# anshulahuja98/antidote

Measured on AMD Instinct MI355X. Metric: materialized ops/sec + VC compares/sec (1/2/4/8 GPU), % of HBM roofline, higher is better.
Workload: dtype u64; 1 GPU; cfg2 counter_pn materialize: 10M keys x 64 ops/key, 8-DC clocks, random snapshot VCs; keys_per_gpu=10000000, keys_total=10000000, ops_per_key=64, n_dcs=8, r_jitter=U[-2000,2000], partitioning=vnode p = key mod 64, gpu = p mod G; no collective, parallelism=dp1

## Files before the change

### antidote_amd/_abi.py

```python
from __future__ import annotations

import ctypes as C

ABI_VERSION = 7

OK = 0
EINVAL, EHIP, ENOMEM, ECAPACITY, ENOTSUP, ERCCL, ENODEV = -1, -2, -3, -4, -5, -6, -7

COUNTER_PN, SET_AW, REGISTER_MV = 1, 2, 3
TYPE_MIXED = 0xFF
EFFECT_INVALID = -(1 << 63)
TAG_INVALID = 0xFFFFFFFF

F_NEWSS, F_CT_IGNORE, F_ERR_UNEXPECTED, F_ERR_CORRUPTED, F_ERR_CAPACITY = 0x1, 0x2, 0x4, 0x8, 0x10
F_CT_FULL = 0x20
HINT_R_FULL, HINT_CT_FLAG, HINT_MIXED = 0x1, 0x2, 0x4
OPS_THRESHOLD = 50
RESIZE_THRESHOLD = 5
GC_ALL_PRUNED = 0x1
UNIQUE_ID_BYTES = 128
U64_MAX = (1 << 64) - 1

TYPE_NAMES = {
    COUNTER_PN: "antidote_crdt_counter_pn",
# ... 105 lines not shown
    "agn_dev_alloc": (C.c_int, [P, C.c_size_t, C.POINTER(P)]),
    "agn_dev_free": (C.c_int, [P, P]),
    "agn_memcpy_h2d": (C.c_int, [P, P, P, C.c_size_t, P]),
    "agn_memcpy_d2h": (C.c_int, [P, P, P, C.c_size_t, P]),
    "agn_memset_d": (C.c_int, [P, P, C.c_int, C.c_size_t, P]),
    "agn_stream_sync": (C.c_int, [P, P]),
    "agn_materialize": (C.c_int, [P, C.POINTER(AgnLog), C.POINTER(AgnRead),
                                  C.POINTER(AgnResult), P]),
    "agn_materialize_host": (C.c_int, [P, C.POINTER(AgnLog), C.POINTER(AgnRead),
                                       C.POINTER(AgnResult)]),
    "agn_state_capacity": (C.c_int, [C.POINTER(AgnLog), C.POINTER(AgnRead), P]),
    "agn_log_index_ids": (C.c_int, [P, C.POINTER(AgnLog), P, P]),
    "agn_log_index_masks": (C.c_int, [P, C.POINTER(AgnLog), P, P]),
    "agn_log_index_pack": (C.c_int, [P, C.POINTER(AgnLog), P, P, P, C.POINTER(C.c_uint64), P]),
    "agn_log_index_pack16": (C.c_int, [P, C.POINTER(AgnLog), P, P, C.POINTER(C.c_uint64), P]),
    "agn_tune": (C.c_int, [P, C.POINTER(AgnLog), C.POINTER(AgnRead), C.POINTER(AgnResult), P,
                           C.c_int, C.POINTER(C.c_int), P]),
    "agn_select_base": (C.c_int, [P, C.c_uint32, C.c_uint64, P, P, P, P, P, P, P, P]),
    "agn_gst_min": (C.c_int, [P, C.c_uint32, C.c_uint64, C.c_uint64, P, P, P, P]),
    "agn_gst_finalize": (C.c_int, [P, C.c_uint32, C.c_uint64, P, P]),
    "agn_update_stable": (C.c_int, [C.c_uint32, P, P, C.POINTER(C.c_int)]),
    "agn_log_ingest": (C.c_int, [P, C.POINTER(AgnLogRecords), C.c_uint32, C.c_uint32,
                                 C.c_uint64, P, P, C.c_uint32, C.POINTER(AgnLog), P, P]),
    "agn_ss_lookup": (C.c_int, [P, C.POINTER(AgnSsCache), C.c_uint64, P, P, P, P, P, P, P, P,
                                P, P]),
    "agn_ss_store": (C.c_int, [P, C.POINTER(AgnSsCache), C.POINTER(AgnLog), C.c_uint64, P, P, P,
                               P, C.POINTER(AgnResult), P, P, P, P, P]),
    "agn_ss_state_compact": (C.c_int, [P, C.POINTER(AgnSsCache), P, P, C.c_uint64, P]),
    "agn_read_cached": (C.c_int, [P, C.POINTER(AgnSsCache), C.POINTER(AgnLog), C.c_uint64, P, P,
                                  P, P, C.POINTER(AgnResult), P, P, P, P]),
# ... 47 lines not shown
    "oracle_select_base": (C.c_int, [C.c_uint32, C.c_uint64, P, P, P, P, P, P, P]),
    "oracle_log_ingest": (C.c_int, [C.POINTER(AgnLogRecords), C.c_uint32, C.c_uint32,
                                    C.c_uint64, P, P, C.c_uint32, C.POINTER(AgnLog)]),
    "oracle_ss_lookup": (C.c_int, [C.POINTER(AgnSsCache), C.c_uint64, P, P, P, P, P, P, P, P,
                                   P]),
    "oracle_ss_store": (C.c_int, [C.POINTER(AgnSsCache), C.POINTER(AgnLog), C.c_uint64, P, P,
                                  P, P, C.POINTER(AgnResult), P, P, P, P]),
    "oracle_prune_ops": (C.c_int, [C.POINTER(AgnLog), P, P, P, C.POINTER(AgnLog), P]),
    "oracle_gst_scalar": (C.c_int, [C.c_uint32, C.c_uint64, P, P]),
    "oracle_dep_check": (C.c_int, [C.c_uint32, C.c_uint64, P, P, P, P, C.c_uint64, P, P, P]),
    "oracle_vc_le": (C.c_int, [C.c_uint32, P, P, P, P]),
    "oracle_vc_all_dots_greater": (C.c_int, [C.c_uint32, P, P, P, P]),
}


ADDITIVE = frozenset({"agn_log_index_pack16"})


def bind(lib, protos):
    for name, (res, args) in protos.items():
        if name in ADDITIVE and not hasattr(lib, name):
            continue
        fn = getattr(lib, name)
        fn.restype = res
        fn.argtypes = args
    return lib
```

### antidote_amd/csrc/api.hip

```cpp
#include <hip/hip_runtime.h>
#include <hipcub/hipcub.hpp>
#include <rccl/rccl.h>

#include <algorithm>
#include <atomic>
#include <cstdarg>
#include <cstdio>
#include <cstdlib>
#include <cstring>
#include <mutex>
#include <string>
#include <thread>
#include <vector>

#include "common.hpp"
#include "gen.hpp"
#include "serve.hpp"

namespace agn {
struct Stager {
    hipStream_t s = nullptr;
    char *d = nullptr, *h = nullptr;
    size_t cap = 0;
};
// ... 125 lines not shown
    std::lock_guard<std::mutex> g(ctx->mi_mu);
    for (const auto &m : ctx->mi)
        if (m.key_mask == log->key_mask && m.n_keys == log->n_keys)
            return many_mixed(m.mixed, m.n_keys);
    return false;
}

namespace {
struct PackEnt {
    agn_ctx *ctx;
    const uint64_t *oc, *key_off;
    uint64_t n_entries, n_keys, seq;
    PackIdx idx;
    bool owned;
    bool owned16;
};
constexpr int kPackIdx = 16;
std::mutex g_pk_mu;
PackEnt g_pk[kPackIdx] = {};
uint64_t g_pk_seq = 0;
std::atomic<int> g_pk_live{0};

void pack_drop16_locked(PackEnt &e) {
    if (e.owned16) {
        (void)hipFree((void *)e.idx.rows16);
        (void)hipFree((void *)e.idx.narrow);
    }
    e.idx.rows16 = nullptr;
    e.idx.narrow = nullptr;
    e.idx.n_wide = 0;
    e.owned16 = false;
}

void pack_drop_locked(PackEnt &e) {
    if (!e.ctx) return;
    pack_drop16_locked(e);
    if (e.owned) {
        (void)hipFree((void *)e.idx.rows);
// ... 17 lines not shown
}

void pack_register(agn_ctx *ctx, const agn_log &log, const PackIdx &idx, bool owned) {
    std::lock_guard<std::mutex> g(g_pk_mu);
    PackEnt *slot = nullptr;
    for (auto &e : g_pk)
        if (pack_match(e, log)) slot = &e;
    for (auto &e : g_pk)
        if (!slot && !e.ctx) slot = &e;
    if (!slot) {
        slot = &g_pk[0];
        for (auto &e : g_pk)
            if (e.seq < slot->seq) slot = &e;
    }
    pack_drop_locked(*slot);
    *slot = {ctx, log.oc, log.key_off, log.n_entries, log.n_keys, ++g_pk_seq, idx, owned, false};
    g_pk_live.fetch_add(1, std::memory_order_release);
}

void pack_unregister16(const agn_log &log) {
    if (g_pk_live.load(std::memory_order_relaxed) == 0) return;
    std::lock_guard<std::mutex> g(g_pk_mu);
    for (auto &e : g_pk)
        if (pack_match(e, log)) pack_drop16_locked(e);
}

bool pack_register16(const agn_log &log, const uint16_t *rows16, const uint8_t *narrow,
                     uint64_t n_wide, bool owned) {
    std::lock_guard<std::mutex> g(g_pk_mu);
    for (auto &e : g_pk)
        if (pack_match(e, log)) {
            pack_drop16_locked(e);
            e.idx.rows16 = rows16;
            e.idx.narrow = narrow;
            e.idx.n_wide = n_wide;
            e.owned16 = owned;
            return true;
        }
    return false;
}

void pack_clear(agn_ctx *ctx) {
    if (g_pk_live.load(std::memory_order_relaxed) == 0) return;
    std::lock_guard<std::mutex> g(g_pk_mu);
    for (auto &e : g_pk)
        if (e.ctx == ctx) pack_drop_locked(e);
}

void pack_forget(const void *p) {
    if (g_pk_live.load(std::memory_order_relaxed) == 0) return;
    std::lock_guard<std::mutex> g(g_pk_mu);
    for (auto &e : g_pk) {
        if (!e.ctx) continue;
        if (p == e.oc || p == e.key_off || p == e.idx.rows || p == e.idx.base || p == e.idx.ok)
            pack_drop_locked(e);
        else if (e.idx.rows16 && (p == e.idx.rows16 || p == e.idx.narrow))
            pack_drop16_locked(e);
    }
}
}

bool pack_lookup(const agn_log &log, PackIdx *out) {
    if (g_pk_live.load(std::memory_order_relaxed) == 0) return false;
    std::lock_guard<std::mutex> g(g_pk_mu);
    for (const auto &e : g_pk)
        if (pack_match(e, log)) {
            *out = e.idx;
            return true;
        }
    return false;
}

// ... 277 lines not shown
    if (log->crdt_type != AGN_COUNTER_PN || log->n_dcs != 8 || log->oc_mask)
        return fail(AGN_ENOTSUP, "index_pack16: counter_pn logs with 8 dense DCs only");
    if (!narrow) return fail(AGN_EINVAL, "index_pack16: narrow required");
    if (((uintptr_t)rows16 & 15u) || misaligned4(narrow))
        return fail(AGN_EINVAL, "index_pack16: rows16 16-byte, narrow 4-byte aligned");
    PackIdx pk{};
    if (!pack_lookup(*log, &pk))
        return fail(AGN_EINVAL, "index_pack16: no packed index registered for the log "
                                "(agn_log_index_pack first)");
    uint64_t wide = 0;
    rc = launch_index_pack16(*log, pk.rows, pk.ok, rows16, narrow, &wide, (hipStream_t)stream);
    if (rc) return rc;
    if (n_wide) *n_wide = wide;
    if (!pack_register16(*log, rows16, narrow, wide, false))
        return fail(AGN_EINVAL, "index_pack16: the log's packed index was dropped meanwhile");
    return AGN_OK;
}

int agn_state_capacity(const agn_log *log, const agn_read *req, uint64_t *cap_off) {
    if (!log || !req || !cap_off) return fail(AGN_EINVAL, "null argument");
    cap_off[0] = 0;
    for (uint64_t i = 0; i < req->n_req; ++i) {
        const uint64_t k = req->keys ? req->keys[i] : i;
        uint64_t c = 0;
        if (log->add_tok)
            for (uint64_t e = log->key_off[k]; e < log->key_off[k] + key_n(log->key_off, log->key_len, k); ++e)
                c += log->add_tok[e] != 0;
        if (req->base_off) c += req->base_off[i + 1] - req->base_off[i];
        else if (req->base_value && is_tag_type(log->crdt_type))
            c += AGN_SS_STATE_PAIRS(req->base_value[i]);
// ... 779 lines not shown
            pack_register(ctx, *log, PackIdx{(uint32_t *)pr, (uint64_t *)pb, (uint8_t *)po}, true);
            void *p16 = nullptr, *pn = nullptr;
            uint64_t wide = 0;
            const bool tier =
                hipMalloc(&p16, E * 8 * sizeof(uint16_t)) == hipSuccess &&
                hipMalloc(&pn, (K + 7) / 8 * 8) == hipSuccess &&
                launch_index_pack16(*log, (const uint32_t *)pr, (const uint8_t *)po, (uint16_t *)p16,
                                    (uint8_t *)pn, &wide, s) == AGN_OK &&
                pack_register16(*log, (const uint16_t *)p16, (const uint8_t *)pn, wide, true);
            if (!tier) {
                (void)hipGetLastError();
                (void)hipStreamSynchronize(s);
                if (p16) (void)hipFree(p16);
                if (pn) (void)hipFree(pn);
            }
        } else {
            (void)hipGetLastError();
            (void)hipStreamSynchronize(s);
            if (pr) (void)hipFree(pr);
            if (pb) (void)hipFree(pb);
            if (po) (void)hipFree(po);
        }
    }
    (void)hipStreamSynchronize(s);
    (void)hipFree(scratch);
    if (he != hipSuccess) err = fail(AGN_EHIP, "k_gen: %s", hipGetErrorString(he));
    if (err) agn_gen_free_dev(ctx, log, req);
    return err;
}

// ... 126 lines not shown
```

### antidote_amd/csrc/common.hpp

```cpp
#pragma once

#include <hip/hip_runtime.h>
#include <stdint.h>
#include <stdlib.h>

#include <atomic>
#include <shared_mutex>

#include "../../include/antidote_gpu.h"

#define AGN_WAVE 64

namespace agn {

extern std::atomic<uint32_t> g_env_gen;
class EnvKnob {
  public:
    explicit EnvKnob(const char *name) : name_(name) {}
    const char *get() {
        const uint32_t g = g_env_gen.load(std::memory_order_acquire);
        if (gen_.load(std::memory_order_acquire) != g) refresh(g);
        return val_.load(std::memory_order_acquire);
    }

// ... 189 lines not shown
                     uint64_t *mixed = nullptr);
void oplog_view(const agn_oplog *L, agn_log *v);
agn_ctx *oplog_ctx(const agn_oplog *L);

int launch_counter(const agn_log &log, const agn_read &req, const agn_result &out,
                   hipStream_t s);
int launch_index_ids(const agn_log &log, uint32_t *out, hipStream_t st);
int launch_index_masks(const agn_log &log, uint64_t *out, uint64_t *mixed, hipStream_t st);
struct PackIdx {
    const uint32_t *rows;
    const uint64_t *base;
    const uint8_t *ok;
    const uint16_t *rows16;
    const uint8_t *narrow;
    uint64_t n_wide;
};
int launch_index_pack(const agn_log &log, uint32_t *rows, uint64_t *base, uint8_t *ok,
                      uint64_t *n_unpacked, hipStream_t st);
int launch_index_pack16(const agn_log &log, const uint32_t *rows, const uint8_t *ok,
                        uint16_t *rows16, uint8_t *narrow, uint64_t *n_wide, hipStream_t st);
bool pack_lookup(const agn_log &log, PackIdx *out);
int launch_counter_dense(const agn_log &log, const agn_read &req, const agn_result &out,
                         hipStream_t s);
int tune_counter_dense(const agn_log &log, const agn_read &req, const agn_result &out,
                       hipStream_t st, int rounds, int *choice, float *ms);
int launch_tags(const agn_log &log, const agn_read &req, const agn_result &out,
                hipStream_t s);
int launch_gst_min(uint32_t D, uint64_t P, uint64_t E, const uint64_t *clocks,
                   const uint8_t *defined, uint64_t *out, hipStream_t s);
int launch_gst_finalize(uint32_t D, uint64_t E, uint64_t *vec, hipStream_t s);
int launch_log_ingest(const agn_log_records &r, uint32_t D, uint64_t n_keys,
                      const uint64_t *max_t, const uint64_t *max_m, uint32_t base,
                      const agn_log &out, uint64_t *totals, hipStream_t st);
int launch_ss_lookup(const agn_ss_cache &c, uint64_t n_req, const uint64_t *keys,
                     const uint64_t *R, const uint64_t *Rm, uint64_t *sct, uint64_t *sctm,
// ... 35 lines not shown
```

### antidote_amd/csrc/counter_scan.hpp

```cpp
#pragma once
#include "common.hpp"

namespace agn {
namespace {

__device__ __forceinline__ uint64_t dpp_u64(uint64_t v, int ctrl_id) {
    uint32_t lo = (uint32_t)v, hi = (uint32_t)(v >> 32);
    switch (ctrl_id) {
        case 0:
            lo = __builtin_amdgcn_update_dpp(0u, lo, 0xB1, 0xF, 0xF, false);
            hi = __builtin_amdgcn_update_dpp(0u, hi, 0xB1, 0xF, 0xF, false);
            break;
        case 1:
            lo = __builtin_amdgcn_update_dpp(0u, lo, 0x4E, 0xF, 0xF, false);
            hi = __builtin_amdgcn_update_dpp(0u, hi, 0x4E, 0xF, 0xF, false);
            break;
        case 2:
            lo = __builtin_amdgcn_update_dpp(0u, lo, 0x141, 0xF, 0xF, false);
            hi = __builtin_amdgcn_update_dpp(0u, hi, 0x141, 0xF, 0xF, false);
            break;
        default:
            lo = __builtin_amdgcn_update_dpp(0u, lo, 0x140, 0xF, 0xF, false);
            hi = __builtin_amdgcn_update_dpp(0u, hi, 0x140, 0xF, 0xF, false);
            break;
// ... 513 lines not shown
        return keep + shfl_xor_u64(send, stride);
    };
    const bool b5 = (lane & 32) != 0, b4 = (lane & 16) != 0, b3 = (lane & 8) != 0;
    uint64_t v4[4], v2[2];
#pragma unroll
    for (int k = 0; k < 4; ++k) v4[k] = xch(b5 ? s[4 + k] : s[k], b5 ? s[k] : s[4 + k], 32);
#pragma unroll
    for (int k = 0; k < 2; ++k) v2[k] = xch(b4 ? v4[2 + k] : v4[k], b4 ? v4[k] : v4[2 + k], 16);
    uint64_t v = xch(b3 ? v2[1] : v2[0], b3 ? v2[0] : v2[1], 8);
    v += dpp_u64(v, 0);
    v += dpp_u64(v, 1);
    v += dpp_u64(v, 2);
    return v;
}

typedef unsigned long long u64x4 __attribute__((ext_vector_type(4)));
typedef u64x4 u64x4_a8 __attribute__((aligned(8)));
typedef u32x4 u32x4_a4 __attribute__((aligned(4)));
__device__ __forceinline__ u64x4 ldc_u64x4(const uint64_t *p) {
    return *(const __attribute__((address_space(4))) u64x4_a8 *)p;
}
__device__ __forceinline__ u32x4 ldc_u32x4(const uint32_t *p) {
    return *(const __attribute__((address_space(4))) u32x4_a4 *)p;
}

template <bool WARM, bool NT, bool EFF_NT = false, bool FROM1 = false>
__device__ __forceinline__ void scan_key_q8(
    const uint64_t *__restrict__ oc, const int64_t *__restrict__ eff,
    const uint64_t *__restrict__ txid, uint64_t txr, uint64_t off, uint64_t n,
    uint64_t n_entries, uint64_t rA, uint64_t rB, uint64_t sA, uint64_t sB, uint64_t &ctA,
// ... 64 lines not shown
```

### antidote_amd/csrc/mat_counter_dense.hip

```cpp
#include <atomic>
#include <cstdlib>
#include <vector>

#include "counter_scan.hpp"

namespace agn {
namespace {

constexpr uint32_t QL_S = 1024, QL_STRIDE = 32;

inline uint32_t counter_order(uint64_t n_req, uint32_t bulk) {
    return order_or(n_req < (1ull << 20) ? 1u : bulk);
}
constexpr uint32_t BULK_CHUNK = 64;
constexpr uint32_t BULK_CHUNK4 = 64;
constexpr bool Q2_FOUR_DEFAULT = true;
constexpr uint32_t BULK_CHUNK8 = 64;
constexpr uint64_t NARROW_WIDE_DIV = 1024;

struct DenseArgs {
    uint64_t n_req;
    uint64_t n_entries;
    uint32_t req_type;
    uint32_t xcd;
    uint32_t pair;
    uint32_t qnt;
    uint32_t hints;
    uint32_t ql_cap;
};

struct MaskArgs {
    const uint64_t *key_mask, *oc_mask, *R_mask, *sct_mask;
    uint64_t *o_mask;
// ... 1117 lines not shown
    const uint64_t left = a.n_req - i0;
    const uint32_t m = left < 4u ? (uint32_t)left : 4u;
#pragma nounroll
    for (uint32_t h = 0; h < m; ++h) q2_serve_oc(a, i0 + h);
}

struct Q2Pack8Params {
    DenseArgs a;
    MaskArgs mk;
    const void *args[20];
    const uint32_t *rows;
    const uint64_t *base;
    const uint8_t *ok;
    const uint16_t *rows16;
    const uint8_t *narrow;
};
static_assert(offsetof(Q2Pack8Params, rows) == offsetof(Q2PackParams, rows) &&
                  offsetof(Q2Pack8Params, base) == offsetof(Q2PackParams, base),
              "Q2Pack8Params extends Q2PackParams");

__global__ __launch_bounds__(64) void k_counter_pack8(Q2Pack8Params) {
    const DenseArgs a = dense_of(kparams<Q2Params>().a);
    const uint32_t blk = block_order(a.xcd, blockIdx.x, gridDim.x);
    const uint64_t i0 = uniform_u64((uint64_t)blk * 8u);
    if (i0 >= a.n_req) return;
    const int lane = lane_id();
    if (i0 + 7u < a.n_req) {
        const auto &pm = kparams<Q2Params>();
        const uint64_t *const key_off = pm.key_off, *const key_len = pm.key_len;
        const uint32_t *const key_id0 = pm.key_id0;
        const uint8_t *const key_type = pm.key_type;
        const uint64_t *const R = pm.R;
        const int64_t *const bvp = pm.base_value;
        const auto &pq = *(const __attribute__((address_space(4))) Q2Pack8Params *)&pm;
        const uint64_t *const pbase = pq.base;
// ... 19 lines not shown
        const uint64_t v_n64 = has_len ? v_lr : v_nx - v_off;
        const uint32_t v_n = (uint32_t)v_n64;
        const uint32_t v_id0 = has_id0 ? v_ir : AGN_ID0_NONE;
        const uint32_t kt = (((lane & 4) ? ktw1 : ktw0) >> (8u * ((uint32_t)lane & 3u))) & 0xffu;
        const uint32_t want = key_type != nullptr ? (a.req_type & 0xffu) : kt;
        const bool lbad = lane < 8 && (v_n64 > (uint64_t)AGN_WAVE || (v_n64 != 0 && kt != want));
        const bool bad = ballot(lbad) != 0ull || nw0 != 0x01010101u || nw1 != 0x01010101u ||
                         a.n_entries == 0;
        if (!bad) {
            const uint16_t *const rows16 = kparams<Q2Pack8Params>().rows16;
            u32x4 c[8];
#pragma unroll
            for (int g = 0; g < 8; ++g)
                c[g] = n8_load_rows<true>(rows16, n8_readlane_u64(v_off, g), a.n_entries);
            const int64_t *const l_eff = kparams<Q2Params>().eff;
            __builtin_amdgcn_sched_barrier(0);
            const uint64_t below = ballot(rv < bv);
            const uint64_t dl = rv - bv;
            const uint32_t tp = n8_thr_pack(dl > 0xFFFFull ? 0xFFFFu : (uint32_t)dl);
            uint32_t v_cnt = 0, v_fx = 0, v_fe = 0, v_inc = 0;
            uint32_t cg = 0;
            const int kg = lane >> 3;
            int64_t ev[8];
#pragma unroll
            for (int g = 0; g < 8; ++g) {
                const uint32_t th0 = __builtin_amdgcn_readlane(tp, 8 * g);
                const uint32_t th1 = __builtin_amdgcn_readlane(tp, 8 * g + 2);
                const uint32_t th2 = __builtin_amdgcn_readlane(tp, 8 * g + 4);
                const uint32_t th3 = __builtin_amdgcn_readlane(tp, 8 * g + 6);
                const uint32_t noR = (uint32_t)(below >> (8 * g)) & 0xFFu;
                const uint32_t n_g = __builtin_amdgcn_readlane(v_n, g);
                const uint64_t off_g = n8_readlane_u64(v_off, g);
                const bool valid = (uint32_t)lane < n_g;
                const bool ex = (noR | n8_excl(c[g], th0, th1, th2, th3)) != 0u;
                const bool mine = valid & !ex;
                const uint64_t exm = ballot(valid & ex);
                const uint32_t cnt = (uint32_t)__builtin_popcountll(ballot(mine));
                const uint32_t fx = exm ? (uint32_t)__builtin_ctzll(exm) : 0xFFFFFFFFu;
                ev[g] = n8_load_eff(l_eff, off_g, mine,
                                    reinterpret_cast<const int64_t *>(R + (i0 + (uint64_t)g) * 8u));
                c[g].x = mine ? c[g].x : 0u;
                c[g].y = mine ? c[g].y : 0u;
                c[g].z = mine ? c[g].z : 0u;
                c[g].w = mine ? c[g].w : 0u;
                v_inc |= mine ? (1u << g) : 0u;
                __builtin_amdgcn_sched_barrier(0);
                cg = kg == g ? cnt : cg;
                v_cnt = put_lane(cnt, g, v_cnt);
                v_fx = put_lane(fx, g, v_fx);
            }
            __builtin_amdgcn_sched_barrier(0);
            const auto &pr = kparams<Q2Params>();
            const uint32_t *const l_op_id = pr.op_id;
            int64_t *const l_value = pr.o_value, *const l_hole = pr.o_hole;
            uint64_t *const l_lastct = pr.o_lastct;
            uint32_t *const l_count = pr.o_count, *const l_flags = pr.o_flags, *const l_err = pr.o_err;
            const int32_t fx = (int32_t)v_fx;
            const uint32_t pos = fx >= 0 ? (uint32_t)fx : v_n - 1u;
            const bool need = lane < 8 && v_id0 == AGN_ID0_NONE && v_n != 0u;
            const uint32_t *const ip = need ? l_op_id + (v_off + (uint64_t)pos)
                                            : reinterpret_cast<const uint32_t *>(R + slot);
            const uint32_t opid = *ip;
            const uint32_t md = n8_maxfold(c);
            const uint64_t ct = cg ? bv + (uint64_t)md : 0ull;
            __builtin_amdgcn_sched_barrier(0);
            uint64_t sm[8];
#pragma unroll
            for (int g = 0; g < 8; ++g) {
                const bool mine = ((v_inc >> g) & 1u) != 0u;
                const bool badv = mine && ev[g] == AGN_EFFECT_INVALID;
                const uint64_t be = ballot(badv);
                v_fe = put_lane(be ? (uint32_t)__builtin_ctzll(be) : 0xFFFFFFFFu, g, v_fe);
                sm[g] = (mine && !badv) ? (uint64_t)ev[g] : 0ull;
            }
            const uint64_t ks = n8_sumfold(sm);
            const uint64_t total =
                ((uint64_t)(uint32_t)__shfl((int)(uint32_t)(ks >> 32), 8 * (int)m8, AGN_WAVE) << 32) |
                (uint32_t)__shfl((int)(uint32_t)ks, 8 * (int)m8, AGN_WAVE);
            __builtin_amdgcn_sched_barrier(0);
            const uint64_t idh = v_id0 != AGN_ID0_NONE ? (uint64_t)v_id0 + (uint64_t)pos : (uint64_t)opid;
            const int64_t hid = v_n ? (int64_t)idh : 0;
            const int32_t fe = (int32_t)v_fe;
            uint32_t fl = v_cnt ? AGN_F_NEWSS : AGN_F_CT_IGNORE;
            fl |= fe >= 0 ? AGN_F_ERR_UNEXPECTED : 0u;
            l_lastct[slot] = ct;
            if (lane < 8) {
                const uint64_t i = i0 + (uint64_t)lane;
                l_value[i] = (int64_t)(reqbase + total);
                l_hole[i] = fx >= 0 ? hid - 1 : hid;
                l_count[i] = v_cnt;
                l_err[i] = fe >= 0 ? (uint32_t)(v_off + (uint64_t)fe) : 0xffffffffu;
                l_flags[i] = fl;
            }
// ... 204 lines not shown
                          (uintptr_t)mk.o_mask;
    const uintptr_t a8 = (uintptr_t)out.count | (uintptr_t)out.flags | (uintptr_t)out.err_pos;
    const bool q2s = ((sv && (sv[0] == '0' || sv[0] == '1')) ? sv[0] == '1' : dflt) &&
                     (a16 & 15u) == 0 && (a8 & 7u) == 0;
    const char *pv = AGN_KNOB("AGN_Q2_PACK");
    const bool pack = dflt && q2e && q2s && log.n_entries != 0 && !(pv && pv[0] == '0') &&
                      pack_lookup(log, &pk);
    const char *fv = AGN_KNOB("AGN_Q2_FOUR");
    const bool four = pack && !req.keys && log.n_entries / 64u <= log.n_keys &&
                      ((fv && (fv[0] == '0' || fv[0] == '1')) ? fv[0] == '1' : Q2_FOUR_DEFAULT);
    const char *nv = AGN_KNOB("AGN_Q2_NARROW");
    const bool eight = four && pk.rows16 && pk.narrow &&
                       ((nv && (nv[0] == '0' || nv[0] == '1'))
                            ? nv[0] == '1'
                            : pk.n_wide * NARROW_WIDE_DIV <= log.n_keys);
    if (eight) {
        a.xcd = counter_order(req.n_req, BULK_CHUNK8);
        const Q2Pack8Params p{a, mk,
                              {req.keys, log.key_off, log.key_len, log.key_type, id0_index(log),
                               log.oc, log.op_id, log.eff, log.txid, req.R, req.sct, req.sct_ignore,
                               req.txid, req.base_value, out.value, out.hole, out.lastct, out.count,
                               out.flags, out.err_pos},
                              pk.rows, pk.base, pk.ok, pk.rows16, pk.narrow};
        hipLaunchKernelGGL(k_counter_pack8, dim3((unsigned)((req.n_req + 7) / 8)), dim3(64), 0, st, p);
    } else if (four) {
        a.xcd = counter_order(req.n_req, BULK_CHUNK4);
        const Q2PackParams p{a, mk,
                             {req.keys, log.key_off, log.key_len, log.key_type, id0_index(log),
                              log.oc, log.op_id, log.eff, log.txid, req.R, req.sct, req.sct_ignore,
                              req.txid, req.base_value, out.value, out.hole, out.lastct, out.count,
                              out.flags, out.err_pos},
                             pk.rows, pk.base, pk.ok};
        hipLaunchKernelGGL(k_counter_pack4, dim3((unsigned)((req.n_req + 3) / 4)), dim3(64), 0, st, p);
    } else if (pack) {
        AGN_Q2L_(false, false, true, true, true);
    } else if (req.sct) {
        if (msk) AGN_Q2L(true, true);
        else AGN_Q2L(true, false);
    } else {
// ... 352 lines not shown
                    u32x4 v;
                    v.x = lo.x | (lo.y << 16);
                    v.y = lo.z | (lo.w << 16);
                    v.z = hh.x | (hh.y << 16);
                    v.w = hh.z | (hh.w << 16);
                    reinterpret_cast<u32x4 *>(rows16)[off + p] = v;
                }
            }
        }
    }
    __syncthreads();
    if (threadIdx.x == 0 && blk_w)
        atomicAdd(&wide[(blockIdx.x % IM_CNT) * IM_STRIDE], (unsigned long long)blk_w);
}

}

int launch_index_pack16(const agn_log &log, const uint32_t *rows, const uint8_t *ok,
                        uint16_t *rows16, uint8_t *narrow, uint64_t *n_wide, hipStream_t st) {
    const uint64_t nb = (log.n_keys + 3) / 4;
    *n_wide = 0;
    if (nb == 0) return AGN_OK;
    if (nb > 0x7fffffffull) return fail(AGN_EINVAL, "index_pack16: too many keys");
    unsigned long long *cnt = nullptr;
    const size_t cb = (size_t)IM_CNT * IM_STRIDE * sizeof(unsigned long long);
    AGN_HIP(pool_malloc(&cnt, cb, st));
    if (hipMemsetAsync(cnt, 0, cb, st) != hipSuccess) {
        (void)hipFreeAsync(cnt, st);
        return fail(AGN_EHIP, "index_pack16: counter reset");
    }
// ... 165 lines not shown
```

### antidote_amd/engine.py

```python
from __future__ import annotations

import ctypes as C
from dataclasses import dataclass, field

import numpy as np

from . import _abi
from ._lib import EngineUnavailable, check, load
from .encode import (EncodedLog, EncodedRead, ResultArrays, alloc_result, log_struct, n_words,
                     read_struct, result_struct)


class DevBuf:

    def __init__(self, eng: "Engine", nbytes: int):
        self.eng, self.nbytes = eng, int(nbytes)
        p = C.c_void_p()
        check(eng.lib.agn_dev_alloc(eng.ctx, self.nbytes, C.byref(p)), "agn_dev_alloc")
        self.ptr = p.value or 0
        eng._bufs.add(self)

    def free(self):
        if self.ptr:
            self.eng.lib.agn_dev_free(self.eng.ctx, self.ptr)
# ... 115 lines not shown
        ls = dlog.struct if isinstance(dlog, DeviceArrays) else dlog
        K, E = int(ls.n_keys), int(ls.n_entries)
        rows16, narrow = self.empty(max(1, E) * 16), self.empty(max(1, (K + 7) // 8) * 8)
        n = C.c_uint64(0)
        check(self.lib.agn_log_index_pack16(self.ctx, C.byref(ls), rows16.ptr, narrow.ptr,
                                            C.byref(n), stream),
              "agn_log_index_pack16")
        if isinstance(dlog, DeviceArrays):
            dlog.bufs.update(pack_rows16=rows16, pack_narrow=narrow)
        return rows16, narrow, n.value

    def drop_pack16(self, dlog):
        ls = dlog.struct if isinstance(dlog, DeviceArrays) else dlog
        check(self.lib.agn_log_index_pack16(self.ctx, C.byref(ls), None, None, None, None),
              "agn_log_index_pack16")

    def drop_pack(self, dlog):
        ls = dlog.struct if isinstance(dlog, DeviceArrays) else dlog
        check(self.lib.agn_log_index_pack(self.ctx, C.byref(ls), None, None, None, None, None),
              "agn_log_index_pack")

    def alloc_log_like(self, log: EncodedLog) -> DeviceArrays:
        s = _abi.AgnLog()
        s.crdt_type, s.n_dcs = log.crdt_type, log.n_dcs
        s.n_keys, s.n_entries = log.n_keys, log.n_entries
        d = DeviceArrays(s)
        for name in ("key_off", "oc", "oc_mask", "op_id", "txid", "eff", "tag", "add_tok",
                     "rem_off", "rem_tok"):
            a = getattr(log, name)
            if a is None or (isinstance(a, np.ndarray) and a.size == 0 and name != "rem_tok"):
# ... 395 lines not shown
```

### include/antidote_gpu.h

```cpp
#ifndef ANTIDOTE_GPU_H
#define ANTIDOTE_GPU_H

#include <stddef.h>
#include <stdint.h>

#ifdef __cplusplus
extern "C" {
#endif

#define AGN_ABI_VERSION 7

#define AGN_OK 0
#define AGN_EINVAL (-1)
#define AGN_EHIP (-2)
#define AGN_ENOMEM (-3)
#define AGN_ECAPACITY (-4)
#define AGN_ENOTSUP (-5)
#define AGN_ERCCL (-6)
#define AGN_ENODEV (-7)

#define AGN_COUNTER_PN 1
#define AGN_SET_AW 2
#define AGN_REGISTER_MV 3
#define AGN_TYPE_MIXED 0xFF
// ... 92 lines not shown
int agn_materialize_host(agn_ctx *ctx, const agn_log *log, const agn_read *req,
                         agn_result *out);

int agn_tune(agn_ctx *ctx, const agn_log *log, const agn_read *req, agn_result *out,
             void *stream, int rounds, int *choice, float *ms);

int agn_log_index_ids(agn_ctx *ctx, const agn_log *log, uint32_t *out, void *stream);

int agn_log_index_masks(agn_ctx *ctx, const agn_log *log, uint64_t *out, void *stream);

int agn_log_index_pack(agn_ctx *ctx, const agn_log *log, uint32_t *rows, uint64_t *base,
                       uint8_t *ok, uint64_t *n_unpacked, void *stream);

int agn_log_index_pack16(agn_ctx *ctx, const agn_log *log, uint16_t *rows16, uint8_t *narrow,
                         uint64_t *n_wide, void *stream);

int agn_state_capacity(const agn_log *host_log, const agn_read *host_req,
                       uint64_t *cap_off);

#define AGN_OPS_THRESHOLD 50
#define AGN_RESIZE_THRESHOLD 5
typedef struct agn_oplog agn_oplog;
int agn_oplog_create(agn_ctx *ctx, uint32_t crdt_type, uint32_t n_dcs, uint64_t n_keys,
                     int sparse, uint32_t init_slots, agn_oplog **out);
int agn_oplog_destroy(agn_oplog *log);
int agn_oplog_append(agn_oplog *log, uint64_t n, const uint64_t *keys, const uint8_t *same_op,
                     const uint64_t *oc, const uint64_t *oc_mask, const uint64_t *txid,
                     const int64_t *eff, const uint32_t *tag, const uint64_t *add_tok,
                     const uint32_t *rem_off, const uint64_t *rem_tok, uint32_t *out_op_id,
                     uint8_t *out_gc_due);
// ... 187 lines not shown
```

Before: 228.9 billion ops/s.

## Add cached int16 effect tier with escape fallback for 8-DC counter materialize

Adds a derived int16 copy of the counter effect column. Values outside ±32767 are marked with a sentinel and counted. The eight-DC packed materialize kernel gets a templated path that loads the 2-byte effects and sums them in 32 bits with a new shuffle/DPP fold. It falls back to the 64-bit effect array only for escaped entries, which also keeps the invalid-effect error check there. The goal is to cut HBM traffic for effects; the cost is an extra index build, a host sync to count escapes, and more registry bookkeeping.

```diff
diff --git a/antidote_amd/_abi.py b/antidote_amd/_abi.py
--- a/antidote_amd/_abi.py
+++ b/antidote_amd/_abi.py
@@ -143,6 +143,7 @@
     "agn_log_index_masks": (C.c_int, [P, C.POINTER(AgnLog), P, P]),
     "agn_log_index_pack": (C.c_int, [P, C.POINTER(AgnLog), P, P, P, C.POINTER(C.c_uint64), P]),
     "agn_log_index_pack16": (C.c_int, [P, C.POINTER(AgnLog), P, P, C.POINTER(C.c_uint64), P]),
+    "agn_log_index_eff16": (C.c_int, [P, C.POINTER(AgnLog), P, C.POINTER(C.c_uint64), P]),
     "agn_tune": (C.c_int, [P, C.POINTER(AgnLog), C.POINTER(AgnRead), C.POINTER(AgnResult), P,
                            C.c_int, C.POINTER(C.c_int), P]),
     "agn_select_base": (C.c_int, [P, C.c_uint32, C.c_uint64, P, P, P, P, P, P, P, P]),
@@ -220,7 +221,7 @@
 }
 
 
-ADDITIVE = frozenset({"agn_log_index_pack16"})
+ADDITIVE = frozenset({"agn_log_index_pack16", "agn_log_index_eff16"})
 
 
 def bind(lib, protos):
diff --git a/antidote_amd/csrc/api.hip b/antidote_amd/csrc/api.hip
--- a/antidote_amd/csrc/api.hip
+++ b/antidote_amd/csrc/api.hip
@@ -163,6 +163,7 @@
     PackIdx idx;
     bool owned;
     bool owned16;
+    bool owned_e;
 };
 constexpr int kPackIdx = 16;
 std::mutex g_pk_mu;
@@ -170,7 +171,16 @@
 uint64_t g_pk_seq = 0;
 std::atomic<int> g_pk_live{0};
 
+void pack_drop_eff_locked(PackEnt &e) {
+    if (e.owned_e) (void)hipFree((void *)e.idx.eff16);
+    e.idx.eff16 = nullptr;
+    e.idx.eff_src = nullptr;
+    e.idx.n_esc = 0;
+    e.owned_e = false;
+}
+
 void pack_drop16_locked(PackEnt &e) {
+    pack_drop_eff_locked(e);
     if (e.owned16) {
         (void)hipFree((void *)e.idx.rows16);
         (void)hipFree((void *)e.idx.narrow);
@@ -218,7 +228,7 @@
             if (e.seq < slot->seq) slot = &e;
     }
     pack_drop_locked(*slot);
-    *slot = {ctx, log.oc, log.key_off, log.n_entries, log.n_keys, ++g_pk_seq, idx, owned, false};
+    *slot = {ctx, log.oc, log.key_off, log.n_entries, log.n_keys, ++g_pk_seq, idx, owned, false, false};
     g_pk_live.fetch_add(1, std::memory_order_release);
 }
 
@@ -244,6 +254,27 @@
     return false;
 }
 
+void pack_unregister_eff(const agn_log &log) {
+    if (g_pk_live.load(std::memory_order_relaxed) == 0) return;
+    std::lock_guard<std::mutex> g(g_pk_mu);
+    for (auto &e : g_pk)
+        if (pack_match(e, log)) pack_drop_eff_locked(e);
+}
+
+bool pack_register_eff(const agn_log &log, const int16_t *eff16, uint64_t n_esc, bool owned) {
+    std::lock_guard<std::mutex> g(g_pk_mu);
+    for (auto &e : g_pk)
+        if (pack_match(e, log) && e.idx.rows16) {
+            pack_drop_eff_locked(e);
+            e.idx.eff16 = eff16;
+            e.idx.eff_src = log.eff;
+            e.idx.n_esc = n_esc;
+            e.owned_e = owned;
+            return true;
+        }
+    return false;
+}
+
 void pack_clear(agn_ctx *ctx) {
     if (g_pk_live.load(std::memory_order_relaxed) == 0) return;
     std::lock_guard<std::mutex> g(g_pk_mu);
@@ -260,6 +291,8 @@
             pack_drop_locked(e);
         else if (e.idx.rows16 && (p == e.idx.rows16 || p == e.idx.narrow))
             pack_drop16_locked(e);
+        else if (e.idx.eff16 && (p == e.idx.eff16 || p == e.idx.eff_src))
+            pack_drop_eff_locked(e);
     }
 }
 }
@@ -567,6 +600,33 @@
     if (n_wide) *n_wide = wide;
     if (!pack_register16(*log, rows16, narrow, wide, false))
         return fail(AGN_EINVAL, "index_pack16: the log's packed index was dropped meanwhile");
+    return AGN_OK;
+}
+
+int agn_log_index_eff16(agn_ctx *ctx, const agn_log *log, int16_t *eff16, uint64_t *n_escaped,
+                        void *stream) {
+    if (!log) return fail(AGN_EINVAL, "index_eff16: null log");
+    int rc = use_device(ctx);
+    if (rc) return rc;
+    if (n_escaped) *n_escaped = 0;
+    if (!eff16) {
+        pack_unregister_eff(*log);
+        return AGN_OK;
+    }
+    if (log->crdt_type != AGN_COUNTER_PN || log->n_dcs != 8 || log->oc_mask)
+        return fail(AGN_ENOTSUP, "index_eff16: counter_pn logs with 8 dense DCs only");
+    if (!log->eff) return fail(AGN_EINVAL, "index_eff16: eff required");
+    if ((uintptr_t)eff16 & 15u) return fail(AGN_EINVAL, "index_eff16: eff16 16-byte aligned");
+    PackIdx pk{};
+    if (!pack_lookup(*log, &pk) || !pk.rows16)
+        return fail(AGN_EINVAL, "index_eff16: no narrow tier registered for the log "
+                                "(agn_log_index_pack16 first)");
+    uint64_t esc = 0;
+    rc = launch_index_eff16(*log, eff16, &esc, (hipStream_t)stream);
+    if (rc) return rc;
+    if (n_escaped) *n_escaped = esc;
+    if (!pack_register_eff(*log, eff16, esc, false))
+        return fail(AGN_EINVAL, "index_eff16: the log's narrow tier was dropped meanwhile");
     return AGN_OK;
 }
 
@@ -1376,6 +1436,17 @@
                 if (p16) (void)hipFree(p16);
                 if (pn) (void)hipFree(pn);
             }
+            void *pe = nullptr;
+            uint64_t esc = 0;
+            const bool etier =
+                tier && hipMalloc(&pe, (E + 7) / 8 * 8 * sizeof(int16_t)) == hipSuccess &&
+                launch_index_eff16(*log, (int16_t *)pe, &esc, s) == AGN_OK &&
+                pack_register_eff(*log, (const int16_t *)pe, esc, true);
+            if (tier && !etier) {
+                (void)hipGetLastError();
+                (void)hipStreamSynchronize(s);
+                if (pe) (void)hipFree(pe);
+            }
         } else {
             (void)hipGetLastError();
             (void)hipStreamSynchronize(s);
diff --git a/antidote_amd/csrc/common.hpp b/antidote_amd/csrc/common.hpp
--- a/antidote_amd/csrc/common.hpp
+++ b/antidote_amd/csrc/common.hpp
@@ -227,11 +227,15 @@
     const uint16_t *rows16;
     const uint8_t *narrow;
     uint64_t n_wide;
+    const int16_t *eff16;
+    const int64_t *eff_src;
+    uint64_t n_esc;
 };
 int launch_index_pack(const agn_log &log, uint32_t *rows, uint64_t *base, uint8_t *ok,
                       uint64_t *n_unpacked, hipStream_t st);
 int launch_index_pack16(const agn_log &log, const uint32_t *rows, const uint8_t *ok,
                         uint16_t *rows16, uint8_t *narrow, uint64_t *n_wide, hipStream_t st);
+int launch_index_eff16(const agn_log &log, int16_t *eff16, uint64_t *n_esc, hipStream_t st);
 bool pack_lookup(const agn_log &log, PackIdx *out);
 int launch_counter_dense(const agn_log &log, const agn_read &req, const agn_result &out,
                          hipStream_t s);
diff --git a/antidote_amd/csrc/counter_scan.hpp b/antidote_amd/csrc/counter_scan.hpp
--- a/antidote_amd/csrc/counter_scan.hpp
+++ b/antidote_amd/csrc/counter_scan.hpp
@@ -551,6 +551,33 @@
     return v;
 }
 
+__device__ __forceinline__ uint32_t n8_load_eff16(const int16_t *__restrict__ eff16, uint64_t off,
+                                                  uint64_t n_entries) {
+    const uint64_t last = n_entries - 1u;
+    const uint64_t o = off < last ? off : last;
+    const uint32_t room = last - o < 63u ? (uint32_t)(last - o) : 63u;
+    const uint32_t l = (uint32_t)lane_id() < room ? (uint32_t)lane_id() : room;
+    return (uint32_t)ld<true>(reinterpret_cast<const uint16_t *>(eff16) + o + l);
+}
+
+__device__ __forceinline__ uint32_t n8_sumfold32(const uint32_t (&s)[8]) {
+    const int lane = lane_id();
+    auto xch = [](uint32_t keep, uint32_t send, int stride) {
+        return keep + (uint32_t)__shfl_xor((int)send, stride, AGN_WAVE);
+    };
+    const bool b5 = (lane & 32) != 0, b4 = (lane & 16) != 0, b3 = (lane & 8) != 0;
+    uint32_t v4[4], v2[2];
+#pragma unroll
+    for (int k = 0; k < 4; ++k) v4[k] = xch(b5 ? s[4 + k] : s[k], b5 ? s[k] : s[4 + k], 32);
+#pragma unroll
+    for (int k = 0; k < 2; ++k) v2[k] = xch(b4 ? v4[2 + k] : v4[k], b4 ? v4[k] : v4[2 + k], 16);
+    uint32_t v = xch(b3 ? v2[1] : v2[0], b3 ? v2[0] : v2[1], 8);
+    v += __builtin_amdgcn_update_dpp(0u, v, 0xB1, 0xF, 0xF, false);
+    v += __builtin_amdgcn_update_dpp(0u, v, 0x4E, 0xF, 0xF, false);
+    v += __builtin_amdgcn_update_dpp(0u, v, 0x141, 0xF, 0xF, false);
+    return v;
+}
+
 typedef unsigned long long u64x4 __attribute__((ext_vector_type(4)));
 typedef u64x4 u64x4_a8 __attribute__((aligned(8)));
 typedef u32x4 u32x4_a4 __attribute__((aligned(4)));
diff --git a/antidote_amd/csrc/mat_counter_dense.hip b/antidote_amd/csrc/mat_counter_dense.hip
--- a/antidote_amd/csrc/mat_counter_dense.hip
+++ b/antidote_amd/csrc/mat_counter_dense.hip
@@ -17,6 +17,8 @@
 constexpr bool Q2_FOUR_DEFAULT = true;
 constexpr uint32_t BULK_CHUNK8 = 64;
 constexpr uint64_t NARROW_WIDE_DIV = 1024;
+constexpr bool EFF16_DEFAULT = true;
+constexpr uint64_t EFF16_ESC_DIV = 1024;
 
 struct DenseArgs {
     uint64_t n_req;
@@ -1164,11 +1166,13 @@
     const uint8_t *ok;
     const uint16_t *rows16;
     const uint8_t *narrow;
+    const int16_t *eff16;
 };
 static_assert(offsetof(Q2Pack8Params, rows) == offsetof(Q2PackParams, rows) &&
                   offsetof(Q2Pack8Params, base) == offsetof(Q2PackParams, base),
               "Q2Pack8Params extends Q2PackParams");
 
+template <bool E16>
 __global__ __launch_bounds__(64) void k_counter_pack8(Q2Pack8Params) {
     const DenseArgs a = dense_of(kparams<Q2Params>().a);
     const uint32_t blk = block_order(a.xcd, blockIdx.x, gridDim.x);
@@ -1218,14 +1222,21 @@
             for (int g = 0; g < 8; ++g)
                 c[g] = n8_load_rows<true>(rows16, n8_readlane_u64(v_off, g), a.n_entries);
             const int64_t *const l_eff = kparams<Q2Params>().eff;
+            uint32_t e16[E16 ? 8 : 1];
+            if constexpr (E16) {
+                const int16_t *const eff16 = kparams<Q2Pack8Params>().eff16;
+#pragma unroll
+                for (int g = 0; g < 8; ++g)
+                    e16[g] = n8_load_eff16(eff16, n8_readlane_u64(v_off, g), a.n_entries);
+            }
             __builtin_amdgcn_sched_barrier(0);
             const uint64_t below = ballot(rv < bv);
             const uint64_t dl = rv - bv;
             const uint32_t tp = n8_thr_pack(dl > 0xFFFFull ? 0xFFFFu : (uint32_t)dl);
-            uint32_t v_cnt = 0, v_fx = 0, v_fe = 0, v_inc = 0;
+            uint32_t v_cnt = 0, v_fx = 0, v_fe = E16 ? 0xFFFFFFFFu : 0u, v_inc = 0;
             uint32_t cg = 0;
             const int kg = lane >> 3;
-            int64_t ev[8];
+            int64_t ev[E16 ? 1 : 8];
 #pragma unroll
             for (int g = 0; g < 8; ++g) {
                 const uint32_t th0 = __builtin_amdgcn_readlane(tp, 8 * g);
@@ -1241,8 +1252,9 @@
                 const uint64_t exm = ballot(valid & ex);
                 const uint32_t cnt = (uint32_t)__builtin_popcountll(ballot(mine));
                 const uint32_t fx = exm ? (uint32_t)__builtin_ctzll(exm) : 0xFFFFFFFFu;
-                ev[g] = n8_load_eff(l_eff, off_g, mine,
-                                    reinterpret_cast<const int64_t *>(R + (i0 + (uint64_t)g) * 8u));
+                if constexpr (!E16)
+                    ev[g] = n8_load_eff(l_eff, off_g, mine,
+                                        reinterpret_cast<const int64_t *>(R + (i0 + (uint64_t)g) * 8u));
                 c[g].x = mine ? c[g].x : 0u;
                 c[g].y = mine ? c[g].y : 0u;
                 c[g].z = mine ? c[g].z : 0u;
@@ -1264,23 +1276,57 @@
             const bool need = lane < 8 && v_id0 == AGN_ID0_NONE && v_n != 0u;
             const uint32_t *const ip = need ? l_op_id + (v_off + (uint64_t)pos)
                                             : reinterpret_cast<const uint32_t *>(R + slot);
-            const uint32_t opid = *ip;
+            uint32_t opid = 0;
+            if (!E16 || ballot(need) != 0ull) opid = *ip;
+            uint32_t v_esc = 0, ks32 = 0;
+            if constexpr (E16) {
+                uint32_t sm[8];
+#pragma unroll
+                for (int g = 0; g < 8; ++g) {
+                    const bool mine = ((v_inc >> g) & 1u) != 0u;
+                    const bool esc = mine && e16[g] == 0x8000u;
+                    v_esc |= esc ? (1u << g) : 0u;
+                    sm[g] = (mine && !esc) ? (uint32_t)(int32_t)(int16_t)e16[g] : 0u;
+                }
+                ks32 = n8_sumfold32(sm);
+                __builtin_amdgcn_sched_barrier(0);
+            }
             const uint32_t md = n8_maxfold(c);
             const uint64_t ct = cg ? bv + (uint64_t)md : 0ull;
             __builtin_amdgcn_sched_barrier(0);
-            uint64_t sm[8];
-#pragma unroll
-            for (int g = 0; g < 8; ++g) {
-                const bool mine = ((v_inc >> g) & 1u) != 0u;
-                const bool badv = mine && ev[g] == AGN_EFFECT_INVALID;
-                const uint64_t be = ballot(badv);
-                v_fe = put_lane(be ? (uint32_t)__builtin_ctzll(be) : 0xFFFFFFFFu, g, v_fe);
-                sm[g] = (mine && !badv) ? (uint64_t)ev[g] : 0ull;
+            uint64_t total;
+            if constexpr (E16) {
+                total = (uint64_t)(int64_t)(int32_t)__shfl((int)ks32, 8 * (int)m8, AGN_WAVE);
+                if (ballot(v_esc != 0u) != 0ull) {
+#pragma nounroll
+                    for (int g = 0; g < 8; ++g) {
+                        const bool esc = ((v_esc >> g) & 1u) != 0u;
+                        if (ballot(esc) == 0ull) continue;
+                        const uint64_t off_g = n8_readlane_u64(v_off, g);
+                        int64_t x = 0;
+                        if (esc) x = l_eff[off_g + (uint64_t)lane];
+                        const bool badv = esc && x == AGN_EFFECT_INVALID;
+                        const uint64_t be = ballot(badv);
+                        const uint64_t xs = (uint64_t)wave_sum_dpp(badv ? 0 : x);
+                        v_fe = put_lane(be ? (uint32_t)__builtin_ctzll(be) : 0xFFFFFFFFu, g, v_fe);
+                        total += lane == g ? xs : 0ull;
+                    }
+                }
+            } else {
+                uint64_t sm[8];
+#pragma unroll
+                for (int g = 0; g < 8; ++g) {
+                    const bool mine = ((v_inc >> g) & 1u) != 0u;
+                    const bool badv = mine && ev[g] == AGN_EFFECT_INVALID;
+                    const uint64_t be = ballot(badv);
+                    v_fe = put_lane(be ? (uint32_t)__builtin_ctzll(be) : 0xFFFFFFFFu, g, v_fe);
+                    sm[g] = (mine && !badv) ? (uint64_t)ev[g] : 0ull;
+                }
+                const uint64_t ks = n8_sumfold(sm);
+                total =
+                    ((uint64_t)(uint32_t)__shfl((int)(uint32_t)(ks >> 32), 8 * (int)m8, AGN_WAVE) << 32) |
+                    (uint32_t)__shfl((int)(uint32_t)ks, 8 * (int)m8, AGN_WAVE);
             }
-            const uint64_t ks = n8_sumfold(sm);
-            const uint64_t total =
-                ((uint64_t)(uint32_t)__shfl((int)(uint32_t)(ks >> 32), 8 * (int)m8, AGN_WAVE) << 32) |
-                (uint32_t)__shfl((int)(uint32_t)ks, 8 * (int)m8, AGN_WAVE);
             __builtin_amdgcn_sched_barrier(0);
             const uint64_t idh = v_id0 != AGN_ID0_NONE ? (uint64_t)v_id0 + (uint64_t)pos : (uint64_t)opid;
             const int64_t hid = v_n ? (int64_t)idh : 0;
@@ -1515,6 +1561,11 @@
                        ((nv && (nv[0] == '0' || nv[0] == '1'))
                             ? nv[0] == '1'
                             : pk.n_wide * NARROW_WIDE_DIV <= log.n_keys);
+    const char *xv = AGN_KNOB("AGN_Q2_EFF16");
+    const bool e16 = eight && pk.eff16 && log.eff == pk.eff_src &&
+                     ((xv && (xv[0] == '0' || xv[0] == '1'))
+                          ? xv[0] == '1'
+                          : EFF16_DEFAULT && pk.n_esc * EFF16_ESC_DIV <= log.n_entries);
     if (eight) {
         a.xcd = counter_order(req.n_req, BULK_CHUNK8);
         const Q2Pack8Params p{a, mk,
@@ -1522,8 +1573,10 @@
                                log.oc, log.op_id, log.eff, log.txid, req.R, req.sct, req.sct_ignore,
                                req.txid, req.base_value, out.value, out.hole, out.lastct, out.count,
                                out.flags, out.err_pos},
-                              pk.rows, pk.base, pk.ok, pk.rows16, pk.narrow};
-        hipLaunchKernelGGL(k_counter_pack8, dim3((unsigned)((req.n_req + 7) / 8)), dim3(64), 0, st, p);
+                              pk.rows, pk.base, pk.ok, pk.rows16, pk.narrow, pk.eff16};
+        const dim3 grid((unsigned)((req.n_req + 7) / 8));
+        if (e16) hipLaunchKernelGGL(k_counter_pack8<true>, grid, dim3(64), 0, st, p);
+        else hipLaunchKernelGGL(k_counter_pack8<false>, grid, dim3(64), 0, st, p);
     } else if (four) {
         a.xcd = counter_order(req.n_req, BULK_CHUNK4);
         const Q2PackParams p{a, mk,
@@ -1906,6 +1959,68 @@
         atomicAdd(&wide[(blockIdx.x % IM_CNT) * IM_STRIDE], (unsigned long long)blk_w);
 }
 
+__global__ __launch_bounds__(256) void k_index_eff16(const int64_t *__restrict__ eff,
+                                                    uint64_t n_entries,
+                                                    int16_t *__restrict__ eff16,
+                                                    unsigned long long *__restrict__ escaped) {
+    __shared__ uint32_t blk_e;
+    if (threadIdx.x == 0) blk_e = 0;
+    __syncthreads();
+    auto narrow16 = [](int64_t x, uint32_t &esc) {
+        const bool fits = x >= -32767 && x <= 32767;
+        esc += fits ? 0u : 1u;
+        return fits ? (uint32_t)x & 0xFFFFu : 0x8000u;
+    };
+    uint32_t esc = 0;
+    const uint64_t units = n_entries / 8u, stride = (uint64_t)gridDim.x * 256u;
+    const uint64_t t = (uint64_t)blockIdx.x * 256u + threadIdx.x;
+    for (uint64_t u = t; u < units; u += stride) {
+        int64_t x[8];
+#pragma unroll
+        for (int j = 0; j < 8; ++j) x[j] = eff[u * 8u + (uint64_t)j];
+        uint32_t h[8];
+#pragma unroll
+        for (int j = 0; j < 8; ++j) h[j] = narrow16(x[j], esc);
+        u32x4 v;
+        v.x = h[0] | (h[1] << 16);
+        v.y = h[2] | (h[3] << 16);
+        v.z = h[4] | (h[5] << 16);
+        v.w = h[6] | (h[7] << 16);
+        reinterpret_cast<u32x4 *>(eff16)[u] = v;
+    }
+    const uint64_t e = units * 8u + t;
+    if (e < n_entries) eff16[e] = (int16_t)(uint16_t)narrow16(eff[e], esc);
+    if (esc) atomicAdd(&blk_e, esc);
+    __syncthreads();
+    if (threadIdx.x == 0 && blk_e)
+        atomicAdd(&escaped[(blockIdx.x % IM_CNT) * IM_STRIDE], (unsigned long long)blk_e);
+}
+
+}
+
+int launch_index_eff16(const agn_log &log, int16_t *eff16, uint64_t *n_esc, hipStream_t st) {
+    *n_esc = 0;
+    if (log.n_entries == 0) return AGN_OK;
+    const uint64_t want = (log.n_entries / 8u + 255u) / 256u;
+    const unsigned nb = (unsigned)(want < 1u ? 1u : want > 8192u ? 8192u : want);
+    unsigned long long *cnt = nullptr;
+    const size_t cb = (size_t)IM_CNT * IM_STRIDE * sizeof(unsigned long long);
+    AGN_HIP(pool_malloc(&cnt, cb, st));
+    if (hipMemsetAsync(cnt, 0, cb, st) != hipSuccess) {
+        (void)hipFreeAsync(cnt, st);
+        return fail(AGN_EHIP, "index_eff16: counter reset");
+    }
+    hipLaunchKernelGGL(k_index_eff16, dim3(nb), dim3(256), 0, st, log.eff, log.n_entries, eff16, cnt);
+    int rc = hipGetLastError() == hipSuccess ? AGN_OK : fail(AGN_EHIP, "index_eff16: launch");
+    std::vector<unsigned long long> h((size_t)IM_CNT * IM_STRIDE);
+    if (rc == AGN_OK &&
+        (hipMemcpyAsync(h.data(), cnt, cb, hipMemcpyDeviceToHost, st) != hipSuccess ||
+         hipStreamSynchronize(st) != hipSuccess))
+        rc = fail(AGN_EHIP, "index_eff16: escape count");
+    if (rc == AGN_OK)
+        for (uint32_t i = 0; i < IM_CNT; ++i) *n_esc += h[(size_t)i * IM_STRIDE];
+    (void)hipFreeAsync(cnt, st);
+    return rc;
 }
 
 int launch_index_pack16(const agn_log &log, const uint32_t *rows, const uint8_t *ok,
diff --git a/antidote_amd/engine.py b/antidote_amd/engine.py
--- a/antidote_amd/engine.py
+++ b/antidote_amd/engine.py
@@ -153,6 +153,22 @@
         ls = dlog.struct if isinstance(dlog, DeviceArrays) else dlog
         check(self.lib.agn_log_index_pack16(self.ctx, C.byref(ls), None, None, None, None),
               "agn_log_index_pack16")
+
+    def index_eff16(self, dlog, stream=None):
+        ls = dlog.struct if isinstance(dlog, DeviceArrays) else dlog
+        E = int(ls.n_entries)
+        eff16 = self.empty((max(1, E) + 7) // 8 * 16)
+        n = C.c_uint64(0)
+        check(self.lib.agn_log_index_eff16(self.ctx, C.byref(ls), eff16.ptr, C.byref(n), stream),
+              "agn_log_index_eff16")
+        if isinstance(dlog, DeviceArrays):
+            dlog.bufs.update(pack_eff16=eff16)
+        return eff16, n.value
+
+    def drop_eff16(self, dlog):
+        ls = dlog.struct if isinstance(dlog, DeviceArrays) else dlog
+        check(self.lib.agn_log_index_eff16(self.ctx, C.byref(ls), None, None, None),
+              "agn_log_index_eff16")
 
     def drop_pack(self, dlog):
         ls = dlog.struct if isinstance(dlog, DeviceArrays) else dlog
diff --git a/include/antidote_gpu.h b/include/antidote_gpu.h
--- a/include/antidote_gpu.h
+++ b/include/antidote_gpu.h
@@ -130,6 +130,9 @@
 
 int agn_log_index_pack16(agn_ctx *ctx, const agn_log *log, uint16_t *rows16, uint8_t *narrow,
                          uint64_t *n_wide, void *stream);
+
+int agn_log_index_eff16(agn_ctx *ctx, const agn_log *log, int16_t *eff16,
+                        uint64_t *n_escaped, void *stream);
 
 int agn_state_capacity(const agn_log *host_log, const agn_read *host_req,
                        uint64_t *cap_off);
```

Result: faster. 268.9 billion ops/s, median of 6 (+17.5%).
